# TUMFTM/ORB_SLAM3_RGBL

Hardware: AMD Instinct MI355X
Metric: RGB-L front-end frames/sec (extract+depth+match) (higher is better)
Workload: dtype u8; 1 GPU; KITTI-00 RGB-L cfg2 (synthetic stand-in); nfeatures=2000, levels=8, lidar_points=121600, match=Hamming brute force, frame i vs i+1, upsampling=InverseDilation Diamond 5, inputs=resident in HBM, parallelism=frames/sequences sharded, 1 rank(s), gather=none

## Files before the change

### orb_slam3_rgbl_amd/csrc/extractor.hip

```cpp
#include <math.h>
#include <stdarg.h>
#include <stdlib.h>
#include <string.h>

#include <algorithm>
#include <vector>

#include "brief_pattern.h"
#include "extractor_kernels.h"
#include "octree_labels.h"

namespace rgbl {

static thread_local char g_err[512] = "";
void set_error(const char* fmt, ...) {
  va_list ap;
  va_start(ap, fmt);
  vsnprintf(g_err, sizeof(g_err), fmt, ap);
  va_end(ap);
}
const char* last_error() { return g_err; }

static inline int round_even_f(float v) { return (int)lrintf(v); }
static inline int round_even_d(double v) { return (int)lrint(v); }
// ... 14 lines not shown

using namespace rgbl;

enum StreamId : uint8_t { kMain = 0, kAux, kLvl, kNumStreams };
enum StepKind : uint8_t { kResize = 0, kFast, kGauss, kOctree, kDesc, kPermute, kRecord, kWait };
struct Step { uint8_t kind, stream, mark, flag; int32_t begin, end; };
constexpr int kMaxMarks = 6;

struct Switches {
  bool graph = true;
  bool gauss_wg256 = false;
  bool octree_stamps = false;
  bool octree_no_hist = false;
  bool octree_ldskeys = true;
  int level_split = 3;
  int octree_wg = 0;
  int compact_min_batch = 8;
  bool xcd_map = true;
  int fast_waves = 0;
  int split_pyr_raw = -1;
  int octree_ncap_raw = -1;
  bool dense_raw = true;
  int split_pyr = 0;
  int octree_ncap = 0;
  bool dense = false;
};

struct rgbl_extractor {
  rgbl_extractor_cfg cfg;
  int device = 0;
  Switches sw;
  hipStream_t stream = nullptr;
  hipStream_t own[kNumStreams] = {};
  hipEvent_t marks[kMaxMarks] = {};
  KernelTimer timer;
  int L = 0;
  std::vector<float> scale, inv_scale, sigma2, inv_sigma2;
  std::vector<int> per_level;
  UMax umax;
  std::vector<LevelGeom> geom;
  BlurTiles blur_tiles;
  int max_cell = 0, max_cell_w = 0;
  int cells_frame = 0, kp_frame = 0;
  size_t pyr_frame = 0, slots_frame = 0, keys_frame = 0, nodes_frame = 0, img_frame = 0;
  int img_pitch = 0;
  std::vector<int> group_off;
  LevelGeom* d_geom = nullptr;
  FastCell* d_cells = nullptr;
  CellGroup* d_groups = nullptr;
  GaussTile* d_gtiles = nullptr;
  ResizeTab *d_xtab = nullptr, *d_ytab = nullptr;
  ResizeGroup* d_xgroups = nullptr;
  int32_t* d_xsxa = nullptr;
  uint8_t* d_rootx = nullptr;
  int8_t* d_pattern = nullptr;
  uint8_t *d_img = nullptr, *d_pyr = nullptr, *d_blur = nullptr;
  uint32_t *d_cellcnt = nullptr, *d_slots = nullptr, *d_keys_a = nullptr, *d_keys_b = nullptr;
  QNode *d_list_a = nullptr, *d_list_b = nullptr;
  QDiv* d_div = nullptr;
  uint32_t *d_todo_a = nullptr, *d_todo_b = nullptr, *d_sval = nullptr;
  uint64_t* d_skey = nullptr;
  uint8_t* d_divided = nullptr;
  uint32_t* d_kpkey = nullptr;
  int* d_kpcount = nullptr;
  uint32_t* d_levelcnt = nullptr;
  unsigned long long* d_dbg = nullptr;
  rgbl_keypoint* d_tmp_kp = nullptr;
  uint8_t* d_tmp_desc = nullptr;
  std::vector<void*> allocs;
  uint8_t* d_stage = nullptr;
  int* d_err = nullptr;
  int32_t *d_out_n = nullptr, *d_out_mono = nullptr;
  rgbl_keypoint* d_out_kp = nullptr;
  uint8_t* d_out_desc = nullptr;
  int out_cap = 0;
  uint8_t* h_pinned = nullptr;
  size_t h_pinned_bytes = 0;
  void* d_color = nullptr;
  size_t color_bytes = 0;
  void* d_rect = nullptr;
  size_t rect_bytes = 0;
  int32_t* d_stereo_sad = nullptr;
  size_t stereo_sad_count = 0;
  void* d_stereo_stage = nullptr;
  size_t stereo_stage_bytes = 0;
  uint8_t* h_stereo_stage = nullptr;
#ifndef RGBL_EMU
  hipGraphExec_t graph_exec = nullptr;
#endif
  int graph_batch = 0, graph_stride = 0, graph_lap0 = 0, graph_lap1 = 0;
  hipStream_t graph_stream = nullptr;
  bool graph_ok = true;
  bool dense_dirty = false;
  struct { bool active = false; const uint8_t* img = nullptr; int w = 0, h = 0, stride = 0, lap0 = 0, lap1 = 0; } pending;
  const uint8_t* last_img0 = nullptr;
  int last_pitch0 = 0;
  size_t last_frame0 = 0;
  int last_batch = 0;
};

namespace {

template <class T>
int dev_alloc(rgbl_extractor* e, T** p, size_t count) {
  RGBL_HIP(hipMalloc(p, std::max<size_t>(count, 1) * sizeof(T)));
  e->allocs.push_back((void*)*p);
// ... 195 lines not shown
  std::vector<GaussTile> gtiles((size_t)e->blur_tiles.tile_off[L]);
  for (int l = 0; l < L; ++l) {
    const LevelGeom& g = e->geom[l];
    const int tx_n = e->blur_tiles.tiles_x[l], n = e->blur_tiles.tile_off[l + 1] - e->blur_tiles.tile_off[l];
    for (int t = 0; t < n; ++t) {
      GaussTile gt;
      memset(&gt, 0, sizeof(gt));
      gt.x0 = (uint16_t)((t % tx_n) * kBlurTW); gt.y0 = (uint16_t)((t / tx_n) * kBlurTH);
      gt.w = (uint16_t)g.w; gt.h = (uint16_t)g.h; gt.pitch = (uint16_t)g.pitch; gt.l = (uint8_t)l; gt.img_off = g.img_off;
      gtiles[(size_t)e->blur_tiles.tile_off[l] + t] = gt;
    }
  }
  RGBL_TRY(dev_alloc(e, &e->d_gtiles, gtiles.size()));
  RGBL_HIP(hipMemcpy(e->d_gtiles, gtiles.data(), sizeof(GaussTile) * gtiles.size(), hipMemcpyHostToDevice));
  RGBL_TRY(dev_alloc(e, &e->d_cells, cells.size()));
  RGBL_HIP(hipMemcpy(e->d_cells, cells.data(), sizeof(FastCell) * cells.size(), hipMemcpyHostToDevice));
  {
    std::vector<CellGroup> groups;
    e->group_off.assign(L + 1, 0);
    for (int l = 0; l < L; ++l) {
      const LevelGeom& g = e->geom[l];
      e->group_off[l] = (int)groups.size();
      for (int ci = 0; ci < g.n_cells; ci += kCompactCells)
        groups.push_back(CellGroup{(uint32_t)(g.cell_off + ci), (uint32_t)std::min(kCompactCells, g.n_cells - ci)});
    }
    e->group_off[L] = (int)groups.size();
    RGBL_TRY(dev_alloc(e, &e->d_groups, groups.size()));
    RGBL_HIP(hipMemcpy(e->d_groups, groups.data(), sizeof(CellGroup) * groups.size(), hipMemcpyHostToDevice));
  }
  RGBL_TRY(dev_alloc(e, &e->d_geom, L));
  RGBL_TRY(dev_alloc(e, &e->d_xtab, xt.size() + 8));
  RGBL_TRY(dev_alloc(e, &e->d_ytab, yt.size()));
  {
    std::vector<ResizeGroup> groups(xt.size() / 4 + 1);
    std::vector<int32_t> sxas(xt.size() / 4 + 1, -1);
    memset(groups.data(), 0, sizeof(ResizeGroup) * groups.size());
    for (int l = 1; l < L; ++l) {
      const int sw = e->geom[l - 1].w;
      const size_t g0 = e->geom[l].xtab_off / 4, g1 = (l + 1 < L ? e->geom[l + 1].xtab_off : xt.size()) / 4;
      for (size_t G = g0; G < g1; ++G) {
        const ResizeTab* X = xt.data() + 4 * G;
        ResizeGroup& R = groups[G];
        const int sxa = std::min((int)X[0].sofs, sw - 8);
        bool ok = sw >= 8 && sxa >= 0;
        for (int i = 0; i < 4; ++i) {
          ok = ok && X[i].sofs >= sxa && X[i].sofs + 1 - sxa <= 7;
          const uint32_t o = (uint32_t)std::min(std::max(X[i].sofs - sxa, 0), 6);
          R.sel[i] = o | (0x0cu << 8) | ((o + 1) << 16) | (0x0cu << 24);
          R.w[i] = (uint32_t)(uint16_t)X[i].a0 | ((uint32_t)(uint16_t)X[i].a1 << 16);
        }
        sxas[G] = ok ? sxa : -1;
      }
    }
    RGBL_TRY(dev_alloc(e, &e->d_xgroups, groups.size()));
    RGBL_TRY(dev_alloc(e, &e->d_xsxa, sxas.size()));
    RGBL_HIP(hipMemcpy(e->d_xgroups, groups.data(), sizeof(ResizeGroup) * groups.size(), hipMemcpyHostToDevice));
    RGBL_HIP(hipMemcpy(e->d_xsxa, sxas.data(), sizeof(int32_t) * sxas.size(), hipMemcpyHostToDevice));
  }
  RGBL_TRY(dev_alloc(e, &e->d_rootx, rootx.size()));
  RGBL_TRY(dev_alloc(e, &e->d_pattern, 1024));
  RGBL_HIP(hipMemcpy(e->d_geom, e->geom.data(), sizeof(LevelGeom) * L, hipMemcpyHostToDevice));
  if (!xt.empty()) RGBL_HIP(hipMemcpy(e->d_xtab, xt.data(), sizeof(ResizeTab) * xt.size(), hipMemcpyHostToDevice));
  if (!yt.empty()) RGBL_HIP(hipMemcpy(e->d_ytab, yt.data(), sizeof(ResizeTab) * yt.size(), hipMemcpyHostToDevice));
  RGBL_HIP(hipMemcpy(e->d_rootx, rootx.data(), rootx.size(), hipMemcpyHostToDevice));
  RGBL_HIP(hipMemcpy(e->d_pattern, kBriefPattern, 1024, hipMemcpyHostToDevice));
  return RGBL_OK;
}

struct StageLayout { size_t counts, mono, kp, desc, bytes; };
StageLayout stage_layout(const rgbl_extractor* e, int batch) {
  StageLayout s;
  s.counts = 256;
  s.mono = s.counts + sizeof(int32_t) * (size_t)e->cfg.max_batch;
  s.kp = align_up(s.mono + sizeof(int32_t) * (size_t)e->cfg.max_batch, 256);
  s.desc = s.kp + align_up((size_t)batch * e->out_cap * sizeof(rgbl_keypoint), 256);
  s.bytes = s.desc + (size_t)batch * e->out_cap * 32;
  return s;
}

int alloc_scratch(rgbl_extractor* e) {
  const size_t B = (size_t)e->cfg.max_batch;
  RGBL_TRY(dev_alloc(e, &e->d_img, B * e->img_frame + 256));
  RGBL_TRY(dev_alloc(e, &e->d_pyr, B * e->pyr_frame + 256));
  RGBL_TRY(dev_alloc(e, &e->d_blur, B * e->pyr_frame + 256));
  RGBL_TRY(dev_alloc(e, &e->d_cellcnt, B * e->cells_frame));
  RGBL_TRY(dev_alloc(e, &e->d_slots, B * e->slots_frame));
  RGBL_TRY(dev_alloc(e, &e->d_keys_a, B * e->keys_frame));
  RGBL_TRY(dev_alloc(e, &e->d_keys_b, B * e->keys_frame));
  if (e->sw.octree_ncap == 0) {
    RGBL_TRY(dev_alloc(e, &e->d_list_a, B * e->nodes_frame));
    RGBL_TRY(dev_alloc(e, &e->d_list_b, B * e->nodes_frame));
    RGBL_TRY(dev_alloc(e, &e->d_div, B * e->nodes_frame));
    RGBL_TRY(dev_alloc(e, &e->d_todo_a, B * e->nodes_frame));
    RGBL_TRY(dev_alloc(e, &e->d_todo_b, B * e->nodes_frame));
    RGBL_TRY(dev_alloc(e, &e->d_skey, B * e->nodes_frame));
    RGBL_TRY(dev_alloc(e, &e->d_sval, B * e->nodes_frame));
    RGBL_TRY(dev_alloc(e, &e->d_divided, B * e->nodes_frame));
  }
  RGBL_TRY(dev_alloc(e, &e->d_kpkey, B * (size_t)e->kp_frame));
  RGBL_TRY(dev_alloc(e, &e->d_kpcount, B * (size_t)e->L));
  RGBL_TRY(dev_alloc(e, &e->d_levelcnt, 2 * B * (size_t)e->L));
  RGBL_HIP(hipMemset(e->d_levelcnt, 0, 2 * B * (size_t)e->L * sizeof(uint32_t)));
  RGBL_TRY(dev_alloc(e, &e->d_dbg, B * (size_t)e->L * 16));
  RGBL_HIP(hipMemset(e->d_dbg, 0, B * (size_t)e->L * 16 * sizeof(unsigned long long)));
  e->out_cap = e->kp_frame;
  const StageLayout lay = stage_layout(e, (int)B);
// ... 146 lines not shown
                         (size_t)e->cells_frame, e->d_slots, e->slots_frame, e->d_geom, L, e->d_keys_a, e->keys_frame, e->d_levelcnt, g0);
      e->timer.end(st);
    }
  };
  auto launch_gauss = [&](hipStream_t st, int tile_begin, int tile_end) {
    if (tile_end <= tile_begin) return;
    e->timer.begin("k_gauss7", st);
    const bool g128 = !e->sw.gauss_wg256;
    hipLaunchKernelGGL(g128 ? k_gauss7<128> : k_gauss7<256>, xcd_grid(e->sw.xcd_map, tile_end - tile_begin, batch), dim3(g128 ? 128 : 256), 0, st, e->d_gtiles,
                       d_imgs, stride, frame_stride, e->d_pyr, e->pyr_frame, e->d_blur, e->pyr_frame, tile_begin);
    e->timer.end(st);
  };
  OctreeBufs ob;
  ob.cell_cnt = e->d_cellcnt; ob.cells_frame = (size_t)e->cells_frame;
  ob.slots = e->d_slots; ob.slots_frame = e->slots_frame;
  ob.keys_a = e->d_keys_a; ob.keys_b = e->d_keys_b; ob.keys_frame = e->keys_frame;
  ob.list_a = e->d_list_a; ob.list_b = e->d_list_b; ob.div = e->d_div;
  ob.todo_a = e->d_todo_a; ob.todo_b = e->d_todo_b; ob.skey = e->d_skey; ob.sval = e->d_sval;
  ob.divided = e->d_divided; ob.nodes_frame = e->nodes_frame;
  ob.rootx = e->d_rootx;
  ob.kp_key = e->d_kpkey; ob.kp_count = e->d_kpcount; ob.kp_frame = (size_t)e->kp_frame;
  ob.level_cnt = e->sw.dense ? e->d_levelcnt : nullptr;
  ob.level_cnt_last = e->d_levelcnt + (size_t)e->cfg.max_batch * L;
  ob.err = e->d_err;
  ob.dbg = e->sw.octree_stamps ? e->d_dbg : nullptr;
  ob.no_hist = e->sw.octree_no_hist ? 1 : 0;
  const bool narrow = e->sw.octree_wg ? e->sw.octree_wg == kOctNarrow : (long)L * batch >= 1024;
  auto launch_octree = [&](hipStream_t st, int level_begin, int level_end) {
    if (level_end <= level_begin) return;
    e->timer.begin("k_octree", st);
    const dim3 grid(level_end - level_begin, batch);
    if (e->sw.octree_ncap == 0) {
      if (narrow) hipLaunchKernelGGL(k_octree_moving<kOctNarrow>, grid, dim3(kOctNarrow), 0, st, e->d_geom, L, ob, level_begin);
      else hipLaunchKernelGGL(k_octree_moving<kOctWide>, grid, dim3(kOctWide), 0, st, e->d_geom, L, ob, level_begin);
    } else if (e->sw.octree_ncap == 512) {
      if (e->sw.octree_ldskeys && !e->sw.octree_wg && (long)(level_end - level_begin) * batch <= 64)
        hipLaunchKernelGGL((k_octree<1024, 512, kOctKeysLds>), grid, dim3(1024), 0, st, e->d_geom, L, ob, level_begin);
      else if (narrow) hipLaunchKernelGGL((k_octree<kOctNarrow, 512>), grid, dim3(kOctNarrow), 0, st, e->d_geom, L, ob, level_begin);
      else hipLaunchKernelGGL((k_octree<kOctWide, 512>), grid, dim3(kOctWide), 0, st, e->d_geom, L, ob, level_begin);
    } else {
      if (e->sw.octree_wg == kOctNarrow) hipLaunchKernelGGL((k_octree<kOctNarrow, 2048>), grid, dim3(kOctNarrow), 0, st, e->d_geom, L, ob, level_begin);
      else if (e->sw.octree_wg == kOctWide) hipLaunchKernelGGL((k_octree<kOctWide, 2048>), grid, dim3(kOctWide), 0, st, e->d_geom, L, ob, level_begin);
      else hipLaunchKernelGGL((k_octree<1024, 2048>), grid, dim3(1024), 0, st, e->d_geom, L, ob, level_begin);
    }
    e->timer.end(st);
  };
  auto launch_resize = [&](hipStream_t st, int l) {
    const LevelGeom& g = e->geom[l];
    const LevelGeom& p = e->geom[l - 1];
    const uint8_t* src = (l == 1) ? d_imgs : e->d_pyr + p.img_off;
    const int spitch = (l == 1) ? stride : p.pitch;
    const size_t sframe = (l == 1) ? frame_stride : e->pyr_frame;
    e->timer.begin("k_resize_linear", st);
    const int rtx = (g.w + 4 * kResizeLanes - 1) / (4 * kResizeLanes), rty = (g.h + 4 * kResizeRows - 1) / (4 * kResizeRows);
    hipLaunchKernelGGL(k_resize_linear, xcd_grid(e->sw.xcd_map, rtx * rty, batch), dim3(kResizeWG), 0, st, src, spitch, sframe, p.w, p.h, e->d_pyr + g.img_off, g.pitch, e->pyr_frame, g.w, g.h,
                     e->d_xtab + g.xtab_off, e->d_xgroups + g.xtab_off / 4, e->d_xsxa + g.xtab_off / 4, e->d_ytab + g.ytab_off, rtx);
    e->timer.end(st);
  };
  const bool lapping = lap1 >= 19 && lap1 >= lap0;
  rgbl_keypoint* kp_dst = lapping ? e->d_tmp_kp : d_kp;
  uint8_t* desc_dst = lapping ? e->d_tmp_desc : d_desc;
#ifdef RGBL_ORIENT_STAMPS
#define RGBL_OB_DBG_ARG , e->d_dbg
#else
#define RGBL_OB_DBG_ARG
#endif
  auto launch_desc = [&](hipStream_t st, int slot_begin, int slot_end, int write_total) {
    if (slot_end <= slot_begin) return;
    e->timer.begin("k_orient_brief", st);
    hipLaunchKernelGGL(k_orient_brief<256>, xcd_grid(e->sw.xcd_map, (slot_end - slot_begin + 4 * kKpPerWave - 1) / (4 * kKpPerWave), batch), dim3(256), 0, st, e->d_geom, L, e->umax,
                       e->d_pattern, d_imgs, stride, frame_stride, e->d_pyr, e->pyr_frame, e->d_blur, e->pyr_frame,
                       e->d_kpkey, e->d_kpcount, (size_t)e->kp_frame, kp_dst, desc_dst, lapping ? e->out_cap : cap, d_n,
                       lapping ? (int32_t*)nullptr : d_mono, e->d_err, slot_begin, slot_end, write_total RGBL_OB_DBG_ARG);
    e->timer.end(st);
  };
  auto launch_permute = [&](hipStream_t st) {
    if (cap < e->out_cap) {
      set_error("vLappingArea packing needs cap >= %d", e->out_cap);
      return RGBL_ERR_CAPACITY;
    }
    e->timer.begin("k_lapping_permute", st);
    hipLaunchKernelGGL(k_lapping_permute, dim3(batch), dim3(256), 0, st, e->d_tmp_kp, e->d_tmp_desc, e->out_cap, d_kp,
                       d_desc, cap, d_n, (float)lap0, (float)lap1, d_mono);
    e->timer.end(st);
    return RGBL_OK;
  };
  auto cell_at = [&](int l) { return l < L ? (int)e->geom[l].cell_off : e->cells_frame; };
  auto slot_at = [&](int l) { return l < L ? e->geom[l].koff : e->kp_frame; };
  const hipStream_t streams[kNumStreams] = {s, e->own[kAux], e->own[kLvl]};
  const Plan plan = build_plan(e, batch, e->timer.enabled, lapping);
  if (plan.marks > kMaxMarks) { set_error("launch plan uses %d marks, the handle has %d events", plan.marks, kMaxMarks); return RGBL_ERR_INVALID; }
  for (const Step& t : plan.steps) {
    const hipStream_t st = streams[t.stream];
    switch (t.kind) {
      case kResize: for (int l = t.begin; l < t.end; ++l) launch_resize(st, l); break;
      case kFast: launch_fast(st, cell_at(t.begin), cell_at(t.end)); break;
      case kGauss: launch_gauss(st, e->blur_tiles.tile_off[t.begin], e->blur_tiles.tile_off[t.end]); break;
      case kOctree: launch_octree(st, t.begin, t.end); break;
      case kDesc: launch_desc(st, slot_at(t.begin), slot_at(t.end), t.flag); break;
      case kRecord: RGBL_HIP(hipEventRecord(e->marks[t.mark], st)); break;
      case kWait: RGBL_HIP(hipStreamWaitEvent(st, e->marks[t.mark], 0)); break;
      case kPermute: RGBL_TRY(launch_permute(st)); break;
    }
  }
  RGBL_HIP(hipGetLastError());
  e->dense_dirty = false;
  return RGBL_OK;
}

// ... 908 lines not shown
```

### orb_slam3_rgbl_amd/csrc/extractor_kernels.h

```cpp
#pragma once
#include "common.h"
#include "resize_tab.h"
#include "sincos_glibc.h"

namespace rgbl {

constexpr int kMaxLevels = 16;
constexpr int kMaxRoots = 16;
constexpr int kMinBorder = 16;

struct LevelGeom {
  int w, h, pitch;
  uint32_t img_off;
  int quota;
  int kcap, koff;
  int n_cols, n_rows, w_cell, h_cell, max_bx, max_by;
  int n_cells, cell_off, cell_cap;
  uint32_t slot_off;
  uint32_t key_off, key_cap;
  uint32_t node_off, node_cap;
  int n_ini;
  int root_x[kMaxRoots + 1];
  int root_first[kMaxRoots + 1];
  uint32_t m_wcell, m_hcell;
  uint32_t rootx_off;
  uint32_t xtab_off, ytab_off;
  float scale;
  int patch_size;
};

struct UMax { int v[16]; };

constexpr int kBlurTileWLog = 5, kBlurTileHLog = 2;
constexpr int kBlurTileW = 1 << kBlurTileWLog, kBlurTileH = 1 << kBlurTileHLog;
static_assert(kBlurTileW * kBlurTileH == 128 && kBlurTileW >= 16 && kBlurTileH >= 4, "one line per tile; k_gauss7 stores 16-byte row pieces of 4-row blocks");
__host__ __device__ inline uint32_t blur_rows(int h) { return (uint32_t)(h + kBlurTileH - 1) & ~(uint32_t)(kBlurTileH - 1); }
__host__ __device__ inline uint32_t blur_offset(int x, int y, int pitch) {
  return (uint32_t)(y >> kBlurTileHLog) * (uint32_t)(kBlurTileH * pitch) + ((uint32_t)(x >> kBlurTileWLog) << 7) +
         ((uint32_t)(y & (kBlurTileH - 1)) << kBlurTileWLog) + (uint32_t)(x & (kBlurTileW - 1));
}

struct QNode {
  uint16_t x0, x1, y0, y1;
  uint32_t beg;
  uint32_t cnt;
};
struct QDiv { uint32_t c[4]; };

__device__ __forceinline__ uint32_t pack_key(int x, int y, int s) { return (uint32_t)x | ((uint32_t)y << 12) | ((uint32_t)s << 24); }
__device__ __forceinline__ int key_x(uint32_t k) { return (int)(k & 0xfff); }
__device__ __forceinline__ int key_y(uint32_t k) { return (int)((k >> 12) & 0xfff); }
__device__ __forceinline__ int key_s(uint32_t k) { return (int)(k >> 24); }

__device__ __forceinline__ uint32_t load_u32_unaligned(const uint8_t* p) {
  uint32_t v;
  __builtin_memcpy(&v, p, 4);
  return v;
}

constexpr int kResizeRows = 4;
constexpr int kResizeLanes = 32, kResizeWG = kResizeLanes * 4;
struct ResizeGroup { uint32_t sel[4], w[4]; };
static_assert(sizeof(ResizeGroup) == 32, "two 16-byte loads per group");

__global__ __launch_bounds__(kResizeWG) void k_resize_linear(const uint8_t* __restrict__ src, int spitch,
                                                       size_t sframe, int sw, int sh,
                                                       uint8_t* __restrict__ dst, int dpitch, size_t dframe,
                                                       int dw, int dh, const ResizeTab* __restrict__ xtab,
                                                       const ResizeGroup* __restrict__ xgroups, const int32_t* __restrict__ xsxa,
                                                       const ResizeTab* __restrict__ ytab, int tiles_x) {
  const int tx = threadIdx.x % kResizeLanes, ty = threadIdx.x / kResizeLanes;
  const int tile_y = xcd_item() / tiles_x, tile_x = xcd_item() - tile_y * tiles_x;
  const int dx0 = (tile_x * kResizeLanes + tx) * 4;
  const int dy0 = (tile_y * 4 + ty) * kResizeRows;
  if (dy0 >= dh || dx0 >= dw) return;
  const uint8_t* S = src + (size_t)xcd_frame() * sframe;
  uint8_t* D = dst + (size_t)xcd_frame() * dframe + (size_t)dy0 * dpitch;
  const int sxa = xsxa[dx0 >> 2];
  const uint4* g4 = reinterpret_cast<const uint4*>(xgroups + (dx0 >> 2));
  const uint4 gs = g4[0], gw = g4[1];
  ResizeTab ry[kResizeRows];
#pragma unroll
  for (int r = 0; r < kResizeRows; ++r) ry[r] = ytab[imin(dy0 + r, dh - 1)];
  if (sxa >= 0) {
    uint32_t r0l[kResizeRows], r0h[kResizeRows], r1l[kResizeRows], r1h[kResizeRows];
#pragma unroll
    for (int r = 0; r < kResizeRows; ++r) {
      const int sy0 = imin(imax(ry[r].sofs, 0), sh - 1), sy1 = imin(imax(ry[r].sofs + 1, 0), sh - 1);
      const uint8_t* S0 = S + (size_t)sy0 * spitch + sxa;
      const uint8_t* S1 = S + (size_t)sy1 * spitch + sxa;
      r0l[r] = load_u32_unaligned(S0); r0h[r] = load_u32_unaligned(S0 + 4);
      r1l[r] = load_u32_unaligned(S1); r1h[r] = load_u32_unaligned(S1 + 4);
    }
    const uint32_t sel[4] = {gs.x, gs.y, gs.z, gs.w}, wt[4] = {gw.x, gw.y, gw.z, gw.w};
#pragma unroll
    for (int r = 0; r < kResizeRows; ++r) {
      const int b0 = ry[r].a0, b1 = ry[r].a1;
      uint32_t out = 0;
#pragma unroll
      for (int i = 0; i < 4; ++i) {
        const int h0 = (int)udot2(perm_bytes(r0h[r], r0l[r], sel[i]), wt[i], 0u);
        const int h1 = (int)udot2(perm_bytes(r1h[r], r1l[r], sel[i]), wt[i], 0u);
        const int v = (((b0 * (h0 >> 4)) >> 16) + ((b1 * (h1 >> 4)) >> 16) + 2) >> 2;
        out |= (uint32_t)(v & 0xff) << (8 * i);
      }
      if (dy0 + r < dh) *reinterpret_cast<uint32_t*>(D + (size_t)r * dpitch + dx0) = out;
    }
    return;
  }
  ResizeTab rx[4];
  {
    const uint4* t4 = reinterpret_cast<const uint4*>(xtab + dx0);
    const uint4 q0 = t4[0], q1 = t4[1];
    rx[0].sofs = (int)q0.x; rx[0].a0 = (int16_t)(q0.y & 0xffff); rx[0].a1 = (int16_t)(q0.y >> 16);
    rx[1].sofs = (int)q0.z; rx[1].a0 = (int16_t)(q0.w & 0xffff); rx[1].a1 = (int16_t)(q0.w >> 16);
    rx[2].sofs = (int)q1.x; rx[2].a0 = (int16_t)(q1.y & 0xffff); rx[2].a1 = (int16_t)(q1.y >> 16);
    rx[3].sofs = (int)q1.z; rx[3].a0 = (int16_t)(q1.w & 0xffff); rx[3].a1 = (int16_t)(q1.w >> 16);
  }
#pragma unroll
  for (int r = 0; r < kResizeRows; ++r) {
    if (dy0 + r >= dh) break;
    const int sy0 = imin(imax(ry[r].sofs, 0), sh - 1), sy1 = imin(imax(ry[r].sofs + 1, 0), sh - 1);
    const uint8_t* S0 = S + (size_t)sy0 * spitch;
    const uint8_t* S1 = S + (size_t)sy1 * spitch;
    const int b0 = ry[r].a0, b1 = ry[r].a1;
    uint8_t* Dr = D + (size_t)r * dpitch;
    uint32_t out = 0;
#pragma unroll
    for (int i = 0; i < 4; ++i) {
      const int dx = dx0 + i;
      if (dx >= dw) break;
      const int sx = rx[i].sofs, sx1 = imin(sx + 1, sw - 1);
      const int h0 = S0[sx] * rx[i].a0 + S0[sx1] * rx[i].a1;
      const int h1 = S1[sx] * rx[i].a0 + S1[sx1] * rx[i].a1;
      const int v = (((b0 * (h0 >> 4)) >> 16) + ((b1 * (h1 >> 4)) >> 16) + 2) >> 2;
      out |= (uint32_t)(v & 0xff) << (8 * i);
    }
    if (dx0 + 3 < dw) {
      *reinterpret_cast<uint32_t*>(Dr + dx0) = out;
    } else {
      for (int i = 0; dx0 + i < dw; ++i) Dr[dx0 + i] = (uint8_t)(out >> (8 * i));
    }
  }
}

constexpr int kCellMax = 72;
constexpr int kCellSmall = 48;

#define RGBL_RING(c, P, k)                                                                            \
  ((k) == 0 ? (c)[3 * (P)] : (k) == 1 ? (c)[3 * (P) + 1] : (k) == 2 ? (c)[2 * (P) + 2]                \
   : (k) == 3 ? (c)[(P) + 3] : (k) == 4 ? (c)[3] : (k) == 5 ? (c)[-(P) + 3] : (k) == 6 ? (c)[-2 * (P) + 2] \
   : (k) == 7 ? (c)[-3 * (P) + 1] : (k) == 8 ? (c)[-3 * (P)] : (k) == 9 ? (c)[-3 * (P) - 1]           \
   : (k) == 10 ? (c)[-2 * (P) - 2] : (k) == 11 ? (c)[-(P) - 3] : (k) == 12 ? (c)[-3]                  \
   : (k) == 13 ? (c)[(P) - 3] : (k) == 14 ? (c)[2 * (P) - 2] : (c)[3 * (P) - 1])

__device__ __forceinline__ int ring_off(int k, int P) {
  switch (k) {
    case 0: return 3 * P; case 1: return 3 * P + 1; case 2: return 2 * P + 2; case 3: return P + 3;
    case 4: return 3; case 5: return -P + 3; case 6: return -2 * P + 2; case 7: return -3 * P + 1;
    case 8: return -3 * P; case 9: return -3 * P - 1; case 10: return -2 * P - 2; case 11: return -P - 3;
    case 12: return -3; case 13: return P - 3; case 14: return 2 * P - 2; default: return 3 * P - 1;
  }
}

#ifdef RGBL_EMU
__device__ __forceinline__ uint32_t pk_sub_i16(uint32_t a, uint32_t b) { return ((a - b) & 0xffffu) | (((a >> 16) - (b >> 16)) << 16); }
__device__ __forceinline__ uint32_t pk_min_i16(uint32_t a, uint32_t b) {
  const int16_t al = (int16_t)a, bl = (int16_t)b, ah = (int16_t)(a >> 16), bh = (int16_t)(b >> 16);
  return (uint16_t)(al < bl ? al : bl) | ((uint32_t)(uint16_t)(ah < bh ? ah : bh) << 16);
}
__device__ __forceinline__ uint32_t pk_max_i16(uint32_t a, uint32_t b) {
  const int16_t al = (int16_t)a, bl = (int16_t)b, ah = (int16_t)(a >> 16), bh = (int16_t)(b >> 16);
  return (uint16_t)(al > bl ? al : bl) | ((uint32_t)(uint16_t)(ah > bh ? ah : bh) << 16);
}
__device__ __forceinline__ uint32_t pk_swap(uint32_t a) { return (a >> 16) | (a << 16); }
#else
typedef short rgbl_s2 __attribute__((ext_vector_type(2)));
__device__ __forceinline__ rgbl_s2 as_s2(uint32_t a) { rgbl_s2 x; __builtin_memcpy(&x, &a, 4); return x; }
__device__ __forceinline__ uint32_t from_s2(rgbl_s2 x) { uint32_t a; __builtin_memcpy(&a, &x, 4); return a; }
__device__ __forceinline__ uint32_t pk_sub_i16(uint32_t a, uint32_t b) { return from_s2(as_s2(a) - as_s2(b)); }
__device__ __forceinline__ uint32_t pk_min_i16(uint32_t a, uint32_t b) { return from_s2(__builtin_elementwise_min(as_s2(a), as_s2(b))); }
__device__ __forceinline__ uint32_t pk_max_i16(uint32_t a, uint32_t b) { return from_s2(__builtin_elementwise_max(as_s2(a), as_s2(b))); }
__device__ __forceinline__ uint32_t pk_swap(uint32_t a) { return from_s2(as_s2(a).yx); }
#endif

__device__ __forceinline__ uint32_t mul24(uint32_t a, uint32_t b) {
#ifdef RGBL_EMU
  return (a & 0xffffffu) * (b & 0xffffffu);
#else
  uint32_t r;
  asm("v_mul_u32_u24 %0, %1, %2" : "=v"(r) : "v"(a), "s"(b));
  return r;
#endif
}

// ... 380 lines not shown
                                                        const uint32_t* __restrict__ slots, size_t slots_frame,
                                                        const LevelGeom* __restrict__ geom, int n_levels,
                                                        uint32_t* __restrict__ dense_keys, size_t keys_frame,
                                                        uint32_t* __restrict__ level_cnt, int group_begin) {
  __shared__ uint32_t s_pref[kCompactCells + 1];
  __shared__ uint32_t s_scan[8];
  __shared__ uint32_t s_base;
  const int tid = threadIdx.x, f = xcd_frame();
  const CellGroup G = groups[xcd_item() + group_begin];
  const FastCell first = cells[G.first];
  const uint32_t cnt = tid < (int)G.count ? cell_cnt[(size_t)f * cells_frame + G.first + tid] : 0u;
  uint32_t total;
  const uint32_t ex = block_exclusive_scan<uint32_t>(cnt, s_scan, &total);
  s_pref[tid] = ex;
  if (tid == 0) {
    s_pref[kCompactCells] = total;
    s_base = total ? atomicAdd(&level_cnt[(size_t)f * n_levels + first.l], total) : 0u;
  }
  __syncthreads();
  if (total == 0) return;
  const uint32_t* src = slots + (size_t)f * slots_frame + first.slot_base;
  uint32_t* out = dense_keys + (size_t)f * keys_frame + geom[first.l].key_off + s_base;
  const uint32_t cell_cap = first.cell_cap;
  for (uint32_t i = (uint32_t)tid; i < total; i += 256u) {
    uint32_t lo = 0;
#pragma unroll
    for (uint32_t step = kCompactCells / 2; step >= 1; step >>= 1)
      if (s_pref[lo + step] <= i) lo += step;
    out[i] = src[lo * cell_cap + (i - s_pref[lo])];
  }
}

constexpr int kBlurTW = 128, kBlurTH = 32;
struct BlurTiles { int tile_off[kMaxLevels + 1]; int tiles_x[kMaxLevels]; };

struct GaussTile { uint16_t x0, y0, w, h, pitch; uint8_t l, pad; uint32_t img_off; };
static_assert(sizeof(GaussTile) == 16, "one s_load_dwordx4 per tile");

template <int kBit>
__device__ __forceinline__ uint32_t quad_xchg(uint32_t v) {
#ifdef RGBL_EMU
  return (uint32_t)__shfl_xor((int)v, kBit);
#else
  return (uint32_t)__builtin_amdgcn_update_dpp(0, (int)v, kBit == 1 ? 0xB1 : 0x4E, 0xF, 0xF, false);
#endif
}

template <int BS>
__global__ __launch_bounds__(BS) void k_gauss7(const GaussTile* __restrict__ tiles,
                                                    const uint8_t* __restrict__ img0, int pitch0, size_t frame0,
                                                    const uint8_t* __restrict__ pyr, size_t pyr_frame,
                                                    uint8_t* __restrict__ blur, size_t blur_frame, int tile_begin) {
  constexpr int kPairs = (kBlurTH + 6) / 2;
  __shared__ uint32_t s_p[kPairs * kBlurTW];
  const int f = xcd_frame();
  const int tid = threadIdx.x, bx = xcd_item() + tile_begin;
  const GaussTile T = tiles[bx];
  const int x0 = T.x0, y0 = T.y0;
  const uint8_t* img = (T.l == 0) ? img0 + (size_t)f * frame0 : pyr + (size_t)f * pyr_frame + T.img_off;
  const int pitch = (T.l == 0) ? pitch0 : (int)T.pitch;
  const int W = T.w, H = T.h;
  const uint32_t kWA = 18u | (34u << 8) | (48u << 16) | (56u << 24), kWB = 48u | (34u << 8) | (18u << 16);

  auto h_sums = [&](const uint32_t (&w)[2][3], int j, int cg) {
    uint32_t hs[2][4];
#pragma unroll
    for (int rr = 0; rr < 2; ++rr) {
#pragma unroll
      for (int i = 0; i < 4; ++i) {
        const uint32_t lo = i == 3 ? w[rr][1] : align_bytes(w[rr][1], w[rr][0], i + 1);
        const uint32_t hi = i == 3 ? w[rr][2] : align_bytes(w[rr][2], w[rr][1], i + 1);
        hs[rr][i] = udot4(lo, kWA, udot4(hi, kWB, 0u));
      }
    }
    uint4 v;
    v.x = hs[0][0] | (hs[1][0] << 16); v.y = hs[0][1] | (hs[1][1] << 16);
    v.z = hs[0][2] | (hs[1][2] << 16); v.w = hs[0][3] | (hs[1][3] << 16);
    *reinterpret_cast<uint4*>(&s_p[j * kBlurTW + 4 * cg]) = v;
  };
  const bool rows_inside = y0 >= 3 && y0 + kBlurTH + 3 <= H;
  for (int task = tid; task < kPairs * 32; task += BS) {
    const int j = task >> 5, cg = task & 31;
    const int x = x0 + 4 * cg;
    if (x < 4 || x + 8 > W) continue;
    int ya = y0 + 2 * j - 3, yb = ya + 1;
    if (!rows_inside) { ya = reflect101(ya, H); yb = reflect101(yb, H); }
    const uint8_t* row0 = img + __umul24((uint32_t)ya, (uint32_t)pitch) + x;
    const uint8_t* row1 = img + __umul24((uint32_t)yb, (uint32_t)pitch) + x;
    uint32_t w[2][3];
    w[0][0] = load_u32_unaligned(row0 - 4); w[0][1] = load_u32_unaligned(row0); w[0][2] = load_u32_unaligned(row0 + 4);
    w[1][0] = load_u32_unaligned(row1 - 4); w[1][1] = load_u32_unaligned(row1); w[1][2] = load_u32_unaligned(row1 + 4);
    h_sums(w, j, cg);
  }
  {
    const int cg_last = imin(31, (W - 1 - x0) >> 2);
    const int cg_r0 = imax(0, imin(cg_last + 1, ((W - 8 - x0) >> 2) + 1));
    const int n_right = (x0 + 4 * cg_r0 + 8 > W) ? cg_last - cg_r0 + 1 : 0;
    const int n_left = (x0 == 0 && cg_r0 > 0) ? 1 : 0;
    const int n_edge = n_left + n_right;
    for (int task = tid; task < kPairs * n_edge; task += BS) {
      const int j = task / n_edge, e = task - j * n_edge;
      const int cg = e < n_left ? 0 : cg_r0 + (e - n_left);
      const int x = x0 + 4 * cg;
      uint32_t w[2][3];
#pragma unroll
      for (int rr = 0; rr < 2; ++rr) {
        const uint8_t* row = img + __umul24((uint32_t)reflect101(y0 + 2 * j + rr - 3, H), (uint32_t)pitch);
        w[rr][0] = w[rr][1] = w[rr][2] = 0;
#pragma unroll
        for (int k = 0; k < 4; ++k) {
          w[rr][0] |= (uint32_t)row[reflect101(x - 4 + k, W)] << (8 * k);
          w[rr][1] |= (uint32_t)row[reflect101(x + k, W)] << (8 * k);
          w[rr][2] |= (uint32_t)row[reflect101(x + 4 + k, W)] << (8 * k);
        }
      }
      h_sums(w, j, cg);
    }
  }
  __syncthreads();
  for (int item = tid; item < 256; item += BS) {
  const int cg = item & 31, rg = item >> 5;
  uint32_t pv[5][4];
#pragma unroll
  for (int j = 0; j < 5; ++j) {
    const uint4 v = *reinterpret_cast<const uint4*>(&s_p[(2 * rg + j) * kBlurTW + 4 * cg]);
    pv[j][0] = v.x; pv[j][1] = v.y; pv[j][2] = v.z; pv[j][3] = v.w;
  }
  const uint32_t kE0 = 18u | (34u << 16), kE1 = 48u | (56u << 16), kE2 = 48u | (34u << 16), kE3 = 18u;
  const uint32_t kO0 = 18u << 16, kO1 = 34u | (48u << 16), kO2 = 56u | (48u << 16), kO3 = 34u | (18u << 16);
  uint32_t out[4];
#pragma unroll
  for (int o = 0; o < 4; ++o) {
    const int b = o >> 1;
    out[o] = 0;
#pragma unroll
    for (int i = 0; i < 4; ++i) {
      uint32_t acc = 32768u;
      if ((o & 1) == 0) {
        acc = udot2(pv[b][i], kE0, acc); acc = udot2(pv[b + 1][i], kE1, acc);
        acc = udot2(pv[b + 2][i], kE2, acc); acc = udot2(pv[b + 3][i], kE3, acc);
      } else {
        acc = udot2(pv[b][i], kO0, acc); acc = udot2(pv[b + 1][i], kO1, acc);
        acc = udot2(pv[b + 2][i], kO2, acc); acc = udot2(pv[b + 3][i], kO3, acc);
      }
      out[o] = i == 0 ? acc >> 16 : perm_bytes(acc, out[o], i == 1 ? 0x0c0c0600u : i == 2 ? 0x0c060100u : 0x06020100u);
    }
  }
  const int q = cg & 3;
#pragma unroll
  for (int o = 0; o < 4; o += 2) {
    const uint32_t got = quad_xchg<1>((q & 1) ? out[o] : out[o + 1]);
    if (q & 1) out[o] = got; else out[o + 1] = got;
  }
#pragma unroll
  for (int o = 0; o < 2; ++o) {
    const uint32_t got = quad_xchg<2>((q & 2) ? out[o] : out[o + 2]);
    if (q & 2) out[o] = got; else out[o + 2] = got;
  }
  const int x = x0 + 16 * (cg >> 2), y = y0 + 4 * rg + q;
  if (x < W && y < H)
    *reinterpret_cast<uint4*>(blur + (size_t)f * blur_frame + T.img_off + blur_offset(x, y, T.pitch)) = make_uint4(out[0], out[1], out[2], out[3]);
  }
}

struct SortPair { uint64_t k; uint32_t v; };
struct SortView {
  uint64_t* key; uint32_t* val;
  __host__ __device__ SortPair get(int i) const { SortPair p; p.k = key[i]; p.v = val[i]; return p; }
  __host__ __device__ void set(int i, SortPair p) const { key[i] = p.k; val[i] = p.v; }
// ... 1370 lines not shown
```

Before: 156,500 frames/s.

## Widen resize and blur horizontal pass to 8 output pixels per thread

The pyramid resize kernel now has each thread produce 8 output pixels per row instead of 4. It uses a host-precomputed per-pair source window and selector table so one 12-byte load per source row serves both groups, and it falls back to the old 4-wide path when the window does not fit. The Gaussian blur's horizontal pass likewise handles 8 columns per task from a single 16-byte load per row, and its edge path is rewritten to work per row. This cuts the number of global loads and table fetches per output, at the cost of fewer threads per workgroup and more registers per thread.

```diff
diff --git a/orb_slam3_rgbl_amd/csrc/extractor.hip b/orb_slam3_rgbl_amd/csrc/extractor.hip
--- a/orb_slam3_rgbl_amd/csrc/extractor.hip
+++ b/orb_slam3_rgbl_amd/csrc/extractor.hip
@@ -90,6 +90,8 @@
   ResizeTab *d_xtab = nullptr, *d_ytab = nullptr;
   ResizeGroup* d_xgroups = nullptr;
   int32_t* d_xsxa = nullptr;
+  ResizePair* d_xpairs = nullptr;
+  int32_t* d_xwin = nullptr;
   uint8_t* d_rootx = nullptr;
   int8_t* d_pattern = nullptr;
   uint8_t *d_img = nullptr, *d_pyr = nullptr, *d_blur = nullptr;
@@ -391,6 +393,35 @@
         sxas[G] = ok ? sxa : -1;
       }
     }
+    std::vector<ResizePair> pairs(groups.size());
+    std::vector<int32_t> wins(groups.size(), -1);
+    memset(pairs.data(), 0, sizeof(ResizePair) * pairs.size());
+    for (int l = 1; l < L; ++l) {
+      const int sw = e->geom[l - 1].w;
+      const size_t g0 = e->geom[l].xtab_off / 4, g1 = (l + 1 < L ? e->geom[l + 1].xtab_off : xt.size()) / 4;
+      const int ng = (int)(g1 - g0);
+      for (int P = 0; 2 * P < ng; ++P) {
+        const ResizeTab* X = xt.data() + 4 * g0 + 8 * (size_t)P;
+        const int n = std::min(8, 4 * ng - 8 * P);
+        int hi = sw - 12, lo = 0;
+        for (int i = 0; i < n; ++i) {
+          hi = std::min(hi, (int)X[i].sofs - 4 * (i >> 2));
+          lo = std::max(lo, (int)X[i].sofs + 1 - 4 * (i >> 2) - 7);
+        }
+        ResizePair& R = pairs[g0 + P];
+        for (int i = 0; i < 8; ++i) {
+          const ResizeTab& T = X[std::min(i, n - 1)];
+          const uint32_t o = (uint32_t)std::min(std::max((int)T.sofs - hi - 4 * (i >> 2), 0), 6);
+          R.sel[i] = o | (0x0cu << 8) | ((o + 1) << 16) | (0x0cu << 24);
+          R.w[i] = (uint32_t)(uint16_t)T.a0 | ((uint32_t)(uint16_t)T.a1 << 16);
+        }
+        wins[g0 + P] = hi >= lo ? hi : -1;
+      }
+    }
+    RGBL_TRY(dev_alloc(e, &e->d_xpairs, pairs.size()));
+    RGBL_TRY(dev_alloc(e, &e->d_xwin, wins.size()));
+    RGBL_HIP(hipMemcpy(e->d_xpairs, pairs.data(), sizeof(ResizePair) * pairs.size(), hipMemcpyHostToDevice));
+    RGBL_HIP(hipMemcpy(e->d_xwin, wins.data(), sizeof(int32_t) * wins.size(), hipMemcpyHostToDevice));
     RGBL_TRY(dev_alloc(e, &e->d_xgroups, groups.size()));
     RGBL_TRY(dev_alloc(e, &e->d_xsxa, sxas.size()));
     RGBL_HIP(hipMemcpy(e->d_xgroups, groups.data(), sizeof(ResizeGroup) * groups.size(), hipMemcpyHostToDevice));
@@ -643,9 +674,10 @@
     const int spitch = (l == 1) ? stride : p.pitch;
     const size_t sframe = (l == 1) ? frame_stride : e->pyr_frame;
     e->timer.begin("k_resize_linear", st);
-    const int rtx = (g.w + 4 * kResizeLanes - 1) / (4 * kResizeLanes), rty = (g.h + 4 * kResizeRows - 1) / (4 * kResizeRows);
+    const int rtx = (g.w + 8 * kResizeLanes - 1) / (8 * kResizeLanes), rty = (g.h + 4 * kResizeRows - 1) / (4 * kResizeRows);
     hipLaunchKernelGGL(k_resize_linear, xcd_grid(e->sw.xcd_map, rtx * rty, batch), dim3(kResizeWG), 0, st, src, spitch, sframe, p.w, p.h, e->d_pyr + g.img_off, g.pitch, e->pyr_frame, g.w, g.h,
-                     e->d_xtab + g.xtab_off, e->d_xgroups + g.xtab_off / 4, e->d_xsxa + g.xtab_off / 4, e->d_ytab + g.ytab_off, rtx);
+                     e->d_xtab + g.xtab_off, e->d_xgroups + g.xtab_off / 4, e->d_xsxa + g.xtab_off / 4, e->d_xpairs + g.xtab_off / 4,
+                     e->d_xwin + g.xtab_off / 4, e->d_ytab + g.ytab_off, rtx);
     e->timer.end(st);
   };
   const bool lapping = lap1 >= 19 && lap1 >= lap0;
diff --git a/orb_slam3_rgbl_amd/csrc/extractor_kernels.h b/orb_slam3_rgbl_amd/csrc/extractor_kernels.h
--- a/orb_slam3_rgbl_amd/csrc/extractor_kernels.h
+++ b/orb_slam3_rgbl_amd/csrc/extractor_kernels.h
@@ -59,29 +59,19 @@
 }
 
 constexpr int kResizeRows = 4;
-constexpr int kResizeLanes = 32, kResizeWG = kResizeLanes * 4;
+constexpr int kResizeLanes = 16, kResizeWG = kResizeLanes * 4;
 struct ResizeGroup { uint32_t sel[4], w[4]; };
 static_assert(sizeof(ResizeGroup) == 32, "two 16-byte loads per group");
-
-__global__ __launch_bounds__(kResizeWG) void k_resize_linear(const uint8_t* __restrict__ src, int spitch,
-                                                       size_t sframe, int sw, int sh,
-                                                       uint8_t* __restrict__ dst, int dpitch, size_t dframe,
-                                                       int dw, int dh, const ResizeTab* __restrict__ xtab,
-                                                       const ResizeGroup* __restrict__ xgroups, const int32_t* __restrict__ xsxa,
-                                                       const ResizeTab* __restrict__ ytab, int tiles_x) {
-  const int tx = threadIdx.x % kResizeLanes, ty = threadIdx.x / kResizeLanes;
-  const int tile_y = xcd_item() / tiles_x, tile_x = xcd_item() - tile_y * tiles_x;
-  const int dx0 = (tile_x * kResizeLanes + tx) * 4;
-  const int dy0 = (tile_y * 4 + ty) * kResizeRows;
-  if (dy0 >= dh || dx0 >= dw) return;
-  const uint8_t* S = src + (size_t)xcd_frame() * sframe;
-  uint8_t* D = dst + (size_t)xcd_frame() * dframe + (size_t)dy0 * dpitch;
+struct ResizePair { uint32_t sel[8], w[8]; };
+static_assert(sizeof(ResizePair) == 64, "four 16-byte loads per pair");
+
+__device__ __forceinline__ void resize_group(const uint8_t* __restrict__ S, int spitch, int sw, int sh, uint8_t* __restrict__ D, int dpitch,
+                                             int dw, int dh, int dx0, int dy0, const ResizeTab (&ry)[kResizeRows],
+                                             const ResizeTab* __restrict__ xtab, const ResizeGroup* __restrict__ xgroups,
+                                             const int32_t* __restrict__ xsxa) {
   const int sxa = xsxa[dx0 >> 2];
   const uint4* g4 = reinterpret_cast<const uint4*>(xgroups + (dx0 >> 2));
   const uint4 gs = g4[0], gw = g4[1];
-  ResizeTab ry[kResizeRows];
-#pragma unroll
-  for (int r = 0; r < kResizeRows; ++r) ry[r] = ytab[imin(dy0 + r, dh - 1)];
   if (sxa >= 0) {
     uint32_t r0l[kResizeRows], r0h[kResizeRows], r1l[kResizeRows], r1h[kResizeRows];
 #pragma unroll
@@ -141,6 +131,58 @@
     } else {
       for (int i = 0; dx0 + i < dw; ++i) Dr[dx0 + i] = (uint8_t)(out >> (8 * i));
     }
+  }
+}
+
+__global__ __launch_bounds__(kResizeWG) void k_resize_linear(const uint8_t* __restrict__ src, int spitch,
+                                                       size_t sframe, int sw, int sh,
+                                                       uint8_t* __restrict__ dst, int dpitch, size_t dframe,
+                                                       int dw, int dh, const ResizeTab* __restrict__ xtab,
+                                                       const ResizeGroup* __restrict__ xgroups, const int32_t* __restrict__ xsxa,
+                                                       const ResizePair* __restrict__ xpairs, const int32_t* __restrict__ xwin,
+                                                       const ResizeTab* __restrict__ ytab, int tiles_x) {
+  const int tx = threadIdx.x % kResizeLanes, ty = threadIdx.x / kResizeLanes;
+  const int tile_y = xcd_item() / tiles_x, tile_x = xcd_item() - tile_y * tiles_x;
+  const int dx0 = (tile_x * kResizeLanes + tx) * 8;
+  const int dy0 = (tile_y * 4 + ty) * kResizeRows;
+  if (dy0 >= dh || dx0 >= dw) return;
+  const uint8_t* S = src + (size_t)xcd_frame() * sframe;
+  uint8_t* D = dst + (size_t)xcd_frame() * dframe + (size_t)dy0 * dpitch;
+  const int wa = xwin[dx0 >> 3];
+  const uint4* p4 = reinterpret_cast<const uint4*>(xpairs + (dx0 >> 3));
+  const uint4 ps0 = p4[0], ps1 = p4[1], pw0 = p4[2], pw1 = p4[3];
+  ResizeTab ry[kResizeRows];
+#pragma unroll
+  for (int r = 0; r < kResizeRows; ++r) ry[r] = ytab[imin(dy0 + r, dh - 1)];
+  if (wa < 0) {
+    resize_group(S, spitch, sw, sh, D, dpitch, dw, dh, dx0, dy0, ry, xtab, xgroups, xsxa);
+    if (dx0 + 4 < dw) resize_group(S, spitch, sw, sh, D, dpitch, dw, dh, dx0 + 4, dy0, ry, xtab, xgroups, xsxa);
+    return;
+  }
+  uint32_t r0[kResizeRows][3], r1[kResizeRows][3];
+#pragma unroll
+  for (int r = 0; r < kResizeRows; ++r) {
+    const int sy0 = imin(imax(ry[r].sofs, 0), sh - 1), sy1 = imin(imax(ry[r].sofs + 1, 0), sh - 1);
+    __builtin_memcpy(r0[r], S + (size_t)sy0 * spitch + wa, 12);
+    __builtin_memcpy(r1[r], S + (size_t)sy1 * spitch + wa, 12);
+  }
+  const uint32_t sel[8] = {ps0.x, ps0.y, ps0.z, ps0.w, ps1.x, ps1.y, ps1.z, ps1.w};
+  const uint32_t wt[8] = {pw0.x, pw0.y, pw0.z, pw0.w, pw1.x, pw1.y, pw1.z, pw1.w};
+#pragma unroll
+  for (int r = 0; r < kResizeRows; ++r) {
+    const int b0 = ry[r].a0, b1 = ry[r].a1;
+    uint32_t out[2] = {0u, 0u};
+#pragma unroll
+    for (int i = 0; i < 8; ++i) {
+      const int g = i >> 2;
+      const int h0 = (int)udot2(perm_bytes(r0[r][g + 1], r0[r][g], sel[i]), wt[i], 0u);
+      const int h1 = (int)udot2(perm_bytes(r1[r][g + 1], r1[r][g], sel[i]), wt[i], 0u);
+      const int v = (((b0 * (h0 >> 4)) >> 16) + ((b1 * (h1 >> 4)) >> 16) + 2) >> 2;
+      out[g] |= (uint32_t)(v & 0xff) << (8 * (i & 3));
+    }
+    uint2 o;
+    o.x = out[0]; o.y = out[1];
+    if (dy0 + r < dh) *reinterpret_cast<uint2*>(D + (size_t)r * dpitch + dx0) = o;
   }
 }
 
@@ -627,6 +669,7 @@
                                                     const uint8_t* __restrict__ pyr, size_t pyr_frame,
                                                     uint8_t* __restrict__ blur, size_t blur_frame, int tile_begin) {
   constexpr int kPairs = (kBlurTH + 6) / 2;
+  constexpr int kGroups = kBlurTW / 8;
   __shared__ uint32_t s_p[kPairs * kBlurTW];
   const int f = xcd_frame();
   const int tid = threadIdx.x, bx = xcd_item() + tile_begin;
@@ -637,59 +680,52 @@
   const int W = T.w, H = T.h;
   const uint32_t kWA = 18u | (34u << 8) | (48u << 16) | (56u << 24), kWB = 48u | (34u << 8) | (18u << 16);
 
-  auto h_sums = [&](const uint32_t (&w)[2][3], int j, int cg) {
-    uint32_t hs[2][4];
-#pragma unroll
-    for (int rr = 0; rr < 2; ++rr) {
-#pragma unroll
-      for (int i = 0; i < 4; ++i) {
-        const uint32_t lo = i == 3 ? w[rr][1] : align_bytes(w[rr][1], w[rr][0], i + 1);
-        const uint32_t hi = i == 3 ? w[rr][2] : align_bytes(w[rr][2], w[rr][1], i + 1);
-        hs[rr][i] = udot4(lo, kWA, udot4(hi, kWB, 0u));
-      }
-    }
-    uint4 v;
-    v.x = hs[0][0] | (hs[1][0] << 16); v.y = hs[0][1] | (hs[1][1] << 16);
-    v.z = hs[0][2] | (hs[1][2] << 16); v.w = hs[0][3] | (hs[1][3] << 16);
-    *reinterpret_cast<uint4*>(&s_p[j * kBlurTW + 4 * cg]) = v;
+  auto h_row = [&](const uint32_t (&w)[4], uint32_t (&hs)[8]) {
+#pragma unroll
+    for (int i = 0; i < 8; ++i) {
+      const int k = i >> 2, s = (i & 3) + 1;
+      const uint32_t lo = s == 4 ? w[k + 1] : align_bytes(w[k + 1], w[k], s);
+      const uint32_t hi = s == 4 ? w[k + 2] : align_bytes(w[k + 2], w[k + 1], s);
+      hs[i] = udot4(lo, kWA, udot4(hi, kWB, 0u));
+    }
   };
   const bool rows_inside = y0 >= 3 && y0 + kBlurTH + 3 <= H;
-  for (int task = tid; task < kPairs * 32; task += BS) {
-    const int j = task >> 5, cg = task & 31;
-    const int x = x0 + 4 * cg;
-    if (x < 4 || x + 8 > W) continue;
+  for (int task = tid; task < kPairs * kGroups; task += BS) {
+    const int j = task / kGroups, cg = task % kGroups;
+    const int x = x0 + 8 * cg;
+    if (x < 4 || x + 12 > W) continue;
     int ya = y0 + 2 * j - 3, yb = ya + 1;
     if (!rows_inside) { ya = reflect101(ya, H); yb = reflect101(yb, H); }
-    const uint8_t* row0 = img + __umul24((uint32_t)ya, (uint32_t)pitch) + x;
-    const uint8_t* row1 = img + __umul24((uint32_t)yb, (uint32_t)pitch) + x;
-    uint32_t w[2][3];
-    w[0][0] = load_u32_unaligned(row0 - 4); w[0][1] = load_u32_unaligned(row0); w[0][2] = load_u32_unaligned(row0 + 4);
-    w[1][0] = load_u32_unaligned(row1 - 4); w[1][1] = load_u32_unaligned(row1); w[1][2] = load_u32_unaligned(row1 + 4);
-    h_sums(w, j, cg);
+    uint4 q0, q1;
+    __builtin_memcpy(&q0, img + __umul24((uint32_t)ya, (uint32_t)pitch) + x - 4, 16);
+    __builtin_memcpy(&q1, img + __umul24((uint32_t)yb, (uint32_t)pitch) + x - 4, 16);
+    const uint32_t w0[4] = {q0.x, q0.y, q0.z, q0.w}, w1[4] = {q1.x, q1.y, q1.z, q1.w};
+    uint32_t h0[8], h1[8];
+    h_row(w0, h0);
+    h_row(w1, h1);
+    uint4* dst = reinterpret_cast<uint4*>(&s_p[j * kBlurTW + 8 * cg]);
+    dst[0] = make_uint4(h0[0] | (h1[0] << 16), h0[1] | (h1[1] << 16), h0[2] | (h1[2] << 16), h0[3] | (h1[3] << 16));
+    dst[1] = make_uint4(h0[4] | (h1[4] << 16), h0[5] | (h1[5] << 16), h0[6] | (h1[6] << 16), h0[7] | (h1[7] << 16));
   }
   {
-    const int cg_last = imin(31, (W - 1 - x0) >> 2);
-    const int cg_r0 = imax(0, imin(cg_last + 1, ((W - 8 - x0) >> 2) + 1));
-    const int n_right = (x0 + 4 * cg_r0 + 8 > W) ? cg_last - cg_r0 + 1 : 0;
+    const int cg_last = imin(kGroups - 1, (W - 1 - x0) >> 3);
+    const int cg_r0 = imax(0, imin(cg_last + 1, ((W - 12 - x0) >> 3) + 1));
+    const int n_right = (x0 + 8 * cg_r0 + 12 > W) ? cg_last - cg_r0 + 1 : 0;
     const int n_left = (x0 == 0 && cg_r0 > 0) ? 1 : 0;
     const int n_edge = n_left + n_right;
-    for (int task = tid; task < kPairs * n_edge; task += BS) {
-      const int j = task / n_edge, e = task - j * n_edge;
+    uint16_t* s_h = reinterpret_cast<uint16_t*>(s_p);
+    for (int task = tid; task < 2 * kPairs * n_edge; task += BS) {
+      const int r = task / n_edge, e = task - r * n_edge;
       const int cg = e < n_left ? 0 : cg_r0 + (e - n_left);
-      const int x = x0 + 4 * cg;
-      uint32_t w[2][3];
-#pragma unroll
-      for (int rr = 0; rr < 2; ++rr) {
-        const uint8_t* row = img + __umul24((uint32_t)reflect101(y0 + 2 * j + rr - 3, H), (uint32_t)pitch);
-        w[rr][0] = w[rr][1] = w[rr][2] = 0;
-#pragma unroll
-        for (int k = 0; k < 4; ++k) {
-          w[rr][0] |= (uint32_t)row[reflect101(x - 4 + k, W)] << (8 * k);
-          w[rr][1] |= (uint32_t)row[reflect101(x + k, W)] << (8 * k);
-          w[rr][2] |= (uint32_t)row[reflect101(x + 4 + k, W)] << (8 * k);
-        }
-      }
-      h_sums(w, j, cg);
+      const int x = x0 + 8 * cg;
+      const uint32_t ro = __umul24((uint32_t)reflect101(y0 + r - 3, H), (uint32_t)pitch);
+      uint32_t w[4] = {0u, 0u, 0u, 0u};
+#pragma unroll
+      for (int k = 0; k < 15; ++k) w[k >> 2] |= (uint32_t)img[ro + (uint32_t)reflect101(x - 4 + k, W)] << (8 * (k & 3));
+      uint32_t hs[8];
+      h_row(w, hs);
+#pragma unroll
+      for (int i = 0; i < 8; ++i) s_h[2 * ((r >> 1) * kBlurTW + 8 * cg + i) + (r & 1)] = (uint16_t)hs[i];
     }
   }
   __syncthreads();
```

Result: faster. 161,300 frames/s (median of 6 runs) (+3.1%).
